# EnricoMiccoli/nodal

Measured on NVIDIA B200. Metric: unknowns_per_second, higher is better.
Workload: dtype f64

## Files before the change

### nodal_b200/csrc/amg.cu

```cuda
#include <algorithm>
#include <cmath>

#include "amg_host.cuh"

void amg_free_csr(nodal_ctx* ctx, AmgCsr& a) {
    if (a.owned) {
        ctx_pool_free(ctx, const_cast<int32_t*>(a.indptr));
        ctx_pool_free(ctx, const_cast<int32_t*>(a.indices));
        ctx_pool_free(ctx, const_cast<double*>(a.data));
    }
    a = AmgCsr();
}

int amg_aggregate(nodal_ctx* ctx, int rounds, const AmgCsr& A, int32_t nown, int32_t base,
                  int32_t** agg_out, int32_t* nc_out, cudaStream_t st) {
    const int32_t n = A.n;
    AmgScratch<int32_t> match(ctx, n), best(ctx, n);
    AmgScratch<u32> leader(ctx, n);
    if (!match.ptr || !best.ptr || !leader.ptr) return NODAL_CUDA_ERROR;
    const int grid = amg_rows_grid(ctx, n);
    CUDA_TRY(cudaMemsetAsync(match, 0xFF, sizeof(int32_t) * (size_t)n, st));
    for (int r = 0; r < rounds; ++r) {
        amg_propose_kernel<<<grid, AT, 0, st>>>(n, A.indptr, A.indices, A.data, match, best, nown, base);
        KERNEL_CHECK();
        amg_accept_kernel<<<grid, AT, 0, st>>>(n, best, match);
        KERNEL_CHECK();
    }
    int32_t* root = best;
    amg_root_kernel<<<grid, AT, 0, st>>>(n, A.indptr, A.indices, A.data, match, root, leader, nown, base);
    KERNEL_CHECK();
    NODAL_TRY(ctx_reserve(ctx, scan_scratch_bytes(n) + 4096));
    u32* total = carve<u32>(ctx, 16);
    if (!total) return NODAL_CUDA_ERROR;
    NODAL_TRY(scan_exclusive_u32(ctx, leader, leader, n, total, st));
    int32_t* agg = match;
    amg_assign_kernel<<<grid, AT, 0, st>>>(n, root, leader, agg);
    KERNEL_CHECK();
    u32* total_h = reinterpret_cast<u32*>(ctx->pinned);
    CUDA_TRY(cudaMemcpyAsync(total_h, total, sizeof(u32), cudaMemcpyDeviceToHost, st));
    CUDA_TRY(cudaStreamSynchronize(st));
    *nc_out = (int32_t)total_h[0];
    *agg_out = match.keep();
    return NODAL_OK;
}

int amg_transpose_pattern(nodal_ctx* ctx, int32_t n, const int32_t* agg, int32_t** pt_ptr_out,
                          int32_t** pt_idx_out, cudaStream_t st) {
    AmgScratch<u64> keys(ctx, n);
    AmgScratch<double> vals(ctx, n), rhs(ctx, (size_t)n + 1), ones(ctx, n);
    if (!keys.ptr || !vals.ptr || !rhs.ptr || !ones.ptr) return NODAL_CUDA_ERROR;
    const int cb = amg_bit_length(n);
    amg_pt_keys_kernel<<<amg_rows_grid(ctx, n), AT, 0, st>>>(n, agg, cb, keys, vals);
    KERNEL_CHECK();
    int64_t cnt = 0;
    NODAL_TRY(nodal_csr_build(ctx, n, n, cb, reinterpret_cast<uint64_t*>(keys.ptr), vals, rhs, &cnt, st));
    if (cnt != n) {
        nodal_set_error("amg: internal error, P^T has %lld entries for %d rows", (long long)cnt, n);
        return NODAL_CUDA_ERROR;
    }
    AmgScratch<int32_t> pp(ctx, (size_t)n + 1), pi(ctx, n);
    if (!pp.ptr || !pi.ptr) return NODAL_CUDA_ERROR;
    NODAL_TRY(nodal_csr_fetch(ctx, n, n, pp, pi, ones, st));
    *pt_ptr_out = pp.keep();
    *pt_idx_out = pi.keep();
    return NODAL_OK;
}

int amg_members(nodal_ctx* ctx, int32_t n, const int32_t* agg, int32_t nc, int32_t** pt_ptr_out,
                int32_t** pt_idx_out, cudaStream_t st) {
    AmgScratch<u32> cnt(ctx, (size_t)nc + 1), cursor(ctx, (size_t)nc + 1);
    AmgScratch<int32_t> pp(ctx, (size_t)nc + 1), pi(ctx, (size_t)std::max(n, 1));
    if (!cnt.ptr || !cursor.ptr || !pp.ptr || !pi.ptr) return NODAL_CUDA_ERROR;
    CUDA_TRY(cudaMemsetAsync(cnt, 0, sizeof(u32) * ((size_t)nc + 1), st));
    CUDA_TRY(cudaMemsetAsync(cursor, 0, sizeof(u32) * ((size_t)nc + 1), st));
    const int grid = amg_rows_grid(ctx, n);
    amg_count_members_kernel<<<grid, AT, 0, st>>>(n, agg, cnt);
    KERNEL_CHECK();
    NODAL_TRY(ctx_reserve(ctx, scan_scratch_bytes((int64_t)nc + 1) + 4096));
    NODAL_TRY(scan_exclusive_u32(ctx, cnt, reinterpret_cast<u32*>(pp.ptr), (int64_t)nc + 1, nullptr, st));
    amg_place_members_kernel<<<grid, AT, 0, st>>>(n, agg, pp, cursor, pi);
    KERNEL_CHECK();
    amg_sort_members_kernel<<<amg_rows_grid(ctx, nc), AT, 0, st>>>(nc, pp, pi);
    KERNEL_CHECK();
    *pt_ptr_out = pp.keep();
    *pt_idx_out = pi.keep();
    return NODAL_OK;
}

int amg_galerkin_merge(nodal_ctx* ctx, const AmgCsr& A, const int32_t* pt_ptr, const int32_t* pt_idx, int32_t nc,
                       const int32_t* label, int32_t ncol_limit, AmgCsr* out, cudaStream_t st) {
    if (A.nnz >= ((int64_t)1 << 32) - 1) return NODAL_BAD_ARG;
    AmgScratch<u32> bound(ctx, (size_t)nc + 1), kept(ctx, (size_t)nc + 1);
    AmgScratch<int32_t> tmp_cols(ctx, (size_t)std::max<int64_t>(A.nnz, 1)), ip(ctx, (size_t)nc + 1);
    AmgScratch<double> tmp_vals(ctx, (size_t)std::max<int64_t>(A.nnz, 1));
    if (!bound.ptr || !kept.ptr || !tmp_cols.ptr || !tmp_vals.ptr || !ip.ptr) return NODAL_CUDA_ERROR;
    const int grid = amg_rows_grid(ctx, nc);
    CUDA_TRY(cudaMemsetAsync(bound.ptr + nc, 0, sizeof(u32), st));
    CUDA_TRY(cudaMemsetAsync(kept.ptr + nc, 0, sizeof(u32), st));
    amg_merge_bound_kernel<<<grid, AT, 0, st>>>(nc, pt_ptr, pt_idx, A.indptr, bound);
    KERNEL_CHECK();
    NODAL_TRY(ctx_reserve(ctx, scan_scratch_bytes((int64_t)nc + 1) + 4096));
    u32* total = carve<u32>(ctx, 16);
    if (!total) return NODAL_CUDA_ERROR;
    const size_t mark = ctx->arena_used;
    NODAL_TRY(scan_exclusive_u32(ctx, bound, bound, (int64_t)nc + 1, nullptr, st));
    ctx->arena_used = mark;
    amg_merge_rows_kernel<<<grid, AT, 0, st>>>(nc, pt_ptr, pt_idx, A.indptr, A.indices, A.data, label, ncol_limit,
                                               bound, tmp_cols, tmp_vals, kept);
    KERNEL_CHECK();
    NODAL_TRY(scan_exclusive_u32(ctx, kept, reinterpret_cast<u32*>(ip.ptr), (int64_t)nc + 1, total, st));
    u32* total_h = reinterpret_cast<u32*>(ctx->pinned);
    CUDA_TRY(cudaMemcpyAsync(total_h, total, sizeof(u32), cudaMemcpyDeviceToHost, st));
    CUDA_TRY(cudaStreamSynchronize(st));
    const int64_t nnzc = total_h[0];
    AmgScratch<int32_t> ix(ctx, (size_t)std::max<int64_t>(nnzc, 1));
    AmgScratch<double> dv(ctx, (size_t)std::max<int64_t>(nnzc, 1));
    if (!ix.ptr || !dv.ptr) return NODAL_CUDA_ERROR;
    amg_merge_compact_kernel<<<grid, AT, 0, st>>>(nc, bound, ip, tmp_cols, tmp_vals, ix, dv);
    KERNEL_CHECK();
    out->n = nc;
    out->nnz = nnzc;
    out->indptr = ip.keep();
    out->indices = ix.keep();
    out->data = dv.keep();
    out->owned = true;
    return NODAL_OK;
}

namespace {

int rows_grid(const nodal_ctx* ctx, int64_t work) { return amg_rows_grid(ctx, work); }
int sell_grid(const nodal_ctx* ctx, int32_t nslices) { return amg_sell_grid(ctx, nslices); }
int bit_length(int64_t v) { return amg_bit_length(v); }
template <typename T>
T* pool(nodal_ctx* ctx, size_t count) { return amg_pool<T>(ctx, count); }
template <typename T>
using Scratch = AmgScratch<T>;
using Csr = AmgCsr;
void free_csr(nodal_ctx* ctx, Csr& a) { amg_free_csr(ctx, a); }
int aggregate(nodal_amg* h, const Csr& A, int32_t** agg_out, int32_t* nc_out, cudaStream_t st) {
    return amg_aggregate(h->ctx, h->rounds, A, 0x7fffffff, 0, agg_out, nc_out, st);
}

bool sorted_galerkin() {
    static const bool on = getenv("NODAL_AMG_SORT_GALERKIN") != nullptr;
    return on;
}

int galerkin(nodal_amg* h, const Csr& A, const int32_t* agg, int32_t nc, Csr* out, cudaStream_t st) {
    nodal_ctx* ctx = h->ctx;
    if (!sorted_galerkin() && amg_merge_pays(A.nnz, nc)) {
        int32_t *pp = nullptr, *pi = nullptr;
        NODAL_TRY(amg_members(ctx, A.n, agg, nc, &pp, &pi, st));
        const int rc = amg_galerkin_merge(ctx, A, pp, pi, nc, agg, 0x7fffffff, out, st);
        ctx_pool_free(ctx, pp);
        ctx_pool_free(ctx, pi);
        return rc;
    }
    Scratch<u64> keys(ctx, A.nnz);
    Scratch<double> vals(ctx, A.nnz), rhs(ctx, (size_t)nc + 1);
    if (!keys.ptr || !vals.ptr || !rhs.ptr) return NODAL_CUDA_ERROR;
    const int cb = bit_length(nc);
    amg_relabel_kernel<<<rows_grid(ctx, A.n), AT, 0, st>>>(A.n, A.indptr, A.indices, A.data, agg, cb,
                                                         keys, vals);
    KERNEL_CHECK();
    int64_t nnzc = 0;
    NODAL_TRY(nodal_csr_build(ctx, nc, A.nnz, cb, reinterpret_cast<uint64_t*>(keys.ptr), vals, rhs,
                              &nnzc, st));
    Scratch<int32_t> ip(ctx, (size_t)nc + 1), ix(ctx, nnzc);
    Scratch<double> dv(ctx, nnzc);
    if (!ip.ptr || !ix.ptr || !dv.ptr) return NODAL_CUDA_ERROR;
    NODAL_TRY(nodal_csr_fetch(ctx, nc, nnzc, ip, ix, dv, st));
    out->n = nc;
    out->nnz = nnzc;
    out->indptr = ip.keep();
    out->indices = ix.keep();
    out->data = dv.keep();
    out->owned = true;
    return NODAL_OK;
}

int transpose_pattern(nodal_amg* h, AmgLevel& L, cudaStream_t st) {
    if (!sorted_galerkin()) return amg_members(h->ctx, L.n, L.agg, L.nc, &L.pt_ptr, &L.pt_idx, st);
    return amg_transpose_pattern(h->ctx, L.n, L.agg, &L.pt_ptr, &L.pt_idx, st);
}

int invert_coarsest(nodal_amg* h, const AmgLevel& L, cudaStream_t st) {
    nodal_ctx* ctx = h->ctx;
    const int32_t n = L.n;
    const size_t elems = (size_t)n * 2 * n;
    Scratch<double> m0(ctx, elems + 32), m1(ctx, elems);
    if (!m0.ptr || !m1.ptr) return NODAL_CUDA_ERROR;
    int* bad = reinterpret_cast<int*>(m0.ptr + elems);
    CUDA_TRY(cudaMemsetAsync(m0, 0, sizeof(double) * (elems + 32), st));
    amg_dense_init_kernel<<<rows_grid(ctx, n), AT, 0, st>>>(n, L.indptr, L.indices, L.data, m0);
    KERNEL_CHECK();
    double *src = m0.ptr, *dst = m1.ptr;
    const int grid = rows_grid(ctx, (int64_t)elems);
    for (int32_t k = 0; k < n; ++k) {
        amg_gj_step_kernel<<<grid, AT, 0, st>>>(n, k, src, dst, bad);
        KERNEL_CHECK();
        std::swap(src, dst);
    }
    h->inv = pool<double>(ctx, (size_t)n * n);
    if (!h->inv) return NODAL_CUDA_ERROR;
    amg_dense_extract_kernel<<<rows_grid(ctx, (int64_t)n * n), AT, 0, st>>>(n, src, h->inv);
    KERNEL_CHECK();
    int* bad_h = reinterpret_cast<int*>(ctx->pinned);
    CUDA_TRY(cudaMemcpyAsync(bad_h, bad, sizeof(int), cudaMemcpyDeviceToHost, st));
    CUDA_TRY(cudaStreamSynchronize(st));
    if (*bad_h != 0) {
        nodal_set_error("amg: the coarsest operator is not positive definite (pivot %d of %d); "
                        "the matrix is not SPD", *bad_h, n);
        return NODAL_BREAKDOWN;
    }
    return NODAL_OK;
}

int build_hierarchy(nodal_amg* h, int32_t n, int64_t nnz, const int32_t* indptr, const int32_t* indices,
                    const double* data, cudaStream_t st) {
    nodal_ctx* ctx = h->ctx;
    Csr cur;
    cur.n = n; cur.nnz = nnz; cur.indptr = indptr; cur.indices = indices; cur.data = data;
    while (cur.n > h->coarse && (int)h->lv.size() < h->maxlevels) {
        Csr A = cur;
        A.owned = false;
        int32_t* comp = nullptr;
        int rc = NODAL_OK;
        for (int pass = 0; pass < h->passes && rc == NODAL_OK; ++pass) {
            int32_t* agg = nullptr;
            int32_t nc = 0;
            Csr Ac;
            rc = aggregate(h, A, &agg, &nc, st);
            if (rc == NODAL_OK) rc = galerkin(h, A, agg, nc, &Ac, st);
            if (rc == NODAL_OK && comp) {
                amg_compose_kernel<<<rows_grid(ctx, cur.n), AT, 0, st>>>(cur.n, comp, agg);
                ++g_nodal_launches;
                if (cudaGetLastError() != cudaSuccess) {
                    nodal_set_error("amg: amg_compose_kernel launch failed");
                    rc = NODAL_CUDA_ERROR;
                }
            }
            if (!comp) comp = agg;
            else ctx_pool_free(ctx, agg);
            free_csr(ctx, A);
            A = Ac;
        }
        double total_nnz = (double)cur.nnz + (double)A.nnz;
        for (const AmgLevel& P : h->lv) total_nnz += (double)P.nnz;
        const bool too_dense = (double)A.nnz > h->max_fill * (double)cur.nnz ||
                               total_nnz > h->max_complexity * (double)(h->lv.empty() ? cur.nnz : h->lv[0].nnz);
        if (rc != NODAL_OK || (double)A.n > 0.9 * (double)cur.n || too_dense) {
            free_csr(ctx, A);
            ctx_pool_free(ctx, comp);
            if (rc != NODAL_OK) {
                free_csr(ctx, cur);
                return rc;
            }
            break;
        }
        AmgLevel L;
        L.n = cur.n; L.nnz = cur.nnz; L.indptr = cur.indptr; L.indices = cur.indices; L.data = cur.data;
        L.owned = cur.owned;
        L.agg = comp;
        L.nc = A.n;
        h->lv.push_back(L);
        cur = A;
        rc = transpose_pattern(h, h->lv.back(), st);
        if (rc != NODAL_OK) {
            free_csr(ctx, cur);
            return rc;
        }
    }
    AmgLevel L;
    L.n = cur.n; L.nnz = cur.nnz; L.indptr = cur.indptr; L.indices = cur.indices; L.data = cur.data;
    L.owned = cur.owned;
    h->lv.push_back(L);
    for (size_t l = 0; l < h->lv.size(); ++l) {
        AmgLevel& V = h->lv[l];
        NODAL_TRY(sell_from_csr(ctx, V.n, V.nnz, V.indptr, V.indices, V.data, &V.sell, st, nullptr));
        V.x = pool<double>(ctx, V.n);
        V.r = pool<double>(ctx, V.n);
        if (l > 0) V.b = pool<double>(ctx, V.n);
        if (!V.x || !V.r || (l > 0 && !V.b)) return NODAL_CUDA_ERROR;
    }
    if (h->lv.back().n <= h->direct_max) NODAL_TRY(invert_coarsest(h, h->lv.back(), st));
    return NODAL_OK;
}

template <int MODE>
int sell_sweep(const nodal_amg* h, const AmgLevel& V, const double* b, const double* x, double* y,
               double* part, cudaStream_t st) {
    const nodal_sell* m = V.sell;
    amg_sell_kernel<MODE><<<sell_grid(h->ctx, m->nslices), AT, 0, st>>>(
        m->n, m->nslices, m->slice_w, m->cols, m->vals, m->dinv, b, x, h->omega, y, part);
    KERNEL_CHECK();
    return NODAL_OK;
}

template <int MODE>
int cycle_sweep(const nodal_amg* h, const AmgLevel& V, const double* b, const double* xc, double* y,
                cudaStream_t st) {
    const nodal_sell* m = V.sell;
    amg_cycle_sweep_kernel<MODE><<<sell_grid(h->ctx, m->nslices), AT, 0, st>>>(
        m->n, m->nslices, m->slice_w, m->cols, m->vals, m->dinv, b, h->omega, V.agg, xc, h->scale, y);
    KERNEL_CHECK();
    return NODAL_OK;
}

int cycle(const nodal_amg* h, const double* b0, double* z0, cudaStream_t st) {
    const nodal_ctx* ctx = h->ctx;
    const int last = (int)h->lv.size() - 1;
    for (int l = 0; l < last; ++l) {
        const AmgLevel& V = h->lv[l];
        const double* b = l == 0 ? b0 : V.b;
        NODAL_TRY(cycle_sweep<1>(h, V, b, nullptr, V.r, st));
        amg_restrict_kernel<<<rows_grid(ctx, V.nc), AT, 0, st>>>(V.nc, V.pt_ptr, V.pt_idx, V.r,
                                                              h->lv[l + 1].b);
        KERNEL_CHECK();
    }
    {
        const AmgLevel& V = h->lv[last];
        const double* b = last == 0 ? b0 : V.b;
        double* x = last == 0 ? z0 : V.x;
        if (h->inv) amg_gemv_kernel<<<rows_grid(ctx, (int64_t)V.n * 32), AT, 0, st>>>(V.n, h->inv, b, x);
        else amg_jacobi0_kernel<<<rows_grid(ctx, V.n), AT, 0, st>>>(V.n, V.sell->dinv, b, h->omega, x);
        KERNEL_CHECK();
    }
    for (int l = last - 1; l >= 0; --l) {
        const AmgLevel& V = h->lv[l];
        const double* b = l == 0 ? b0 : V.b;
        NODAL_TRY(cycle_sweep<2>(h, V, b, h->lv[l + 1].x, l == 0 ? z0 : V.x, st));
    }
    return NODAL_OK;
}

}

extern "C" int nodal_amg_destroy(nodal_amg* h) {
    if (!h) return NODAL_OK;
    cudaSetDevice(h->device);
    nodal_ctx* ctx = h->ctx;
    for (AmgLevel& V : h->lv) {
        sell_free(V.sell);
        if (V.owned) {
            ctx_pool_free(ctx, const_cast<int32_t*>(V.indptr));
            ctx_pool_free(ctx, const_cast<int32_t*>(V.indices));
            ctx_pool_free(ctx, const_cast<double*>(V.data));
        }
        ctx_pool_free(ctx, V.agg);
        ctx_pool_free(ctx, V.pt_ptr);
        ctx_pool_free(ctx, V.pt_idx);
        ctx_pool_free(ctx, V.b);
        ctx_pool_free(ctx, V.x);
        ctx_pool_free(ctx, V.r);
    }
    ctx_pool_free(ctx, h->inv);
    ctx_pool_free(ctx, h->p);
    ctx_pool_free(ctx, h->q);
    ctx_pool_free(ctx, h->r);
    ctx_pool_free(ctx, h->z);
    ctx_pool_free(ctx, h->part);
    delete h;
    return NODAL_OK;
}

extern "C" int nodal_amg_create(nodal_ctx* ctx, int32_t n, int64_t nnz, const int32_t* indptr,
                                const int32_t* indices, const double* data, const double* params,
                                nodal_amg** out, void* stream) {
    NvtxRange nvtx_range("nodal_amg_create");
    if (!ctx || n < 0 || nnz < 0 || !out) return NODAL_BAD_ARG;
    *out = nullptr;
    cudaStream_t st = (cudaStream_t)stream;
    CUDA_TRY(cudaSetDevice(ctx->device));
    nodal_amg* h = new nodal_amg();
    h->ctx = ctx;
    h->device = ctx->device;
    if (params) {
        if (params[0] >= 1.0) h->passes = (int)params[0];
        if (params[1] >= 1.0) h->coarse = (int)params[1];
        if (params[2] > 0.0) h->omega = params[2];
        if (params[3] > 0.0) h->scale = params[3];
        if (params[4] >= 1.0) h->maxlevels = (int)params[4];
        if (params[5] >= 1.0) h->rounds = (int)params[5];
        if (params[6] >= 1.0) h->direct_max = (int)params[6];
        if (params[7] > 0.0) h->max_fill = params[7];
    }
    cudaEvent_t e0, e1;
    CUDA_TRY(cudaEventCreate(&e0));
    CUDA_TRY(cudaEventCreate(&e1));
    cudaEventRecord(e0, st);
    int rc = NODAL_OK;
    if (n > 0) rc = build_hierarchy(h, n, nnz, indptr, indices, data, st);
    if (rc == NODAL_OK && n > 0) {
        h->nparts = std::max(sell_grid(ctx, h->lv[0].sell->nslices), rows_grid(ctx, n));
        h->p = pool<double>(ctx, n);
        h->q = pool<double>(ctx, n);
        h->r = pool<double>(ctx, n);
        h->z = pool<double>(ctx, n);
        h->part = pool<double>(ctx, 3 * (size_t)h->nparts + 16);
        if (!h->p || !h->q || !h->r || !h->z || !h->part) rc = NODAL_CUDA_ERROR;
    }
    cudaEventRecord(e1, st);
    if (cudaEventSynchronize(e1) == cudaSuccess) cudaEventElapsedTime(&h->setup_ms, e0, e1);
    cudaEventDestroy(e0);
    cudaEventDestroy(e1);
    if (rc != NODAL_OK) {
        nodal_amg_destroy(h);
        return rc;
    }
    *out = h;
    return NODAL_OK;
}

extern "C" int nodal_amg_info(const nodal_amg* h, int32_t cap, int32_t* nlevels, int64_t* rows,
                              int64_t* nnz, double* setup_ms, int32_t* direct) {
    if (!h || !nlevels) return NODAL_BAD_ARG;
    *nlevels = (int32_t)h->lv.size();
    for (int32_t l = 0; l < *nlevels && l < cap; ++l) {
        if (rows) rows[l] = h->lv[l].n;
        if (nnz) nnz[l] = h->lv[l].nnz;
    }
    if (setup_ms) *setup_ms = h->setup_ms;
    if (direct) *direct = h->inv ? 1 : 0;
    return NODAL_OK;
}

extern "C" int nodal_amg_fetch_level(nodal_ctx* ctx, const nodal_amg* h, int32_t level, int32_t* agg,
                                     int32_t* indptr, int32_t* indices, double* data, void* stream) {
    if (!ctx || !h || level < 0 || level >= (int32_t)h->lv.size()) return NODAL_BAD_ARG;
    cudaStream_t st = (cudaStream_t)stream;
    CUDA_TRY(cudaSetDevice(ctx->device));
    const AmgLevel& V = h->lv[level];
    if (agg) {
        if (!V.agg) return NODAL_BAD_ARG;
        CUDA_TRY(cudaMemcpyAsync(agg, V.agg, sizeof(int32_t) * (size_t)V.n, cudaMemcpyDeviceToDevice, st));
    }
    if (indptr) CUDA_TRY(cudaMemcpyAsync(indptr, V.indptr, sizeof(int32_t) * ((size_t)V.n + 1), cudaMemcpyDeviceToDevice, st));
    if (indices) CUDA_TRY(cudaMemcpyAsync(indices, V.indices, sizeof(int32_t) * (size_t)V.nnz, cudaMemcpyDeviceToDevice, st));
    if (data) CUDA_TRY(cudaMemcpyAsync(data, V.data, sizeof(double) * (size_t)V.nnz, cudaMemcpyDeviceToDevice, st));
    return NODAL_OK;
}

extern "C" int nodal_amg_apply(nodal_ctx* ctx, const nodal_amg* h, const double* r, double* z,
                               void* stream) {
    if (!ctx || !h || h->ctx != ctx) return NODAL_BAD_ARG;
    if (h->lv.empty()) return NODAL_OK;
    CUDA_TRY(cudaSetDevice(ctx->device));
    return cycle(h, r, z, (cudaStream_t)stream);
}

extern "C" int nodal_amg_pcg(nodal_ctx* ctx, nodal_amg* h, const double* rhs, double* x, double rtol,
                             int32_t maxit, int32_t* iters_h, double* relres_h, double* stats_h,
                             void* stream) {
    NvtxRange nvtx_range("nodal_amg_pcg");
    if (!ctx || !h || h->ctx != ctx || !iters_h || !relres_h) return NODAL_BAD_ARG;
    *iters_h = 0;
    *relres_h = 0.0;
    if (stats_h) memset(stats_h, 0, 16 * sizeof(double));
    if (h->lv.empty()) return NODAL_OK;
    cudaStream_t st = (cudaStream_t)stream;
    CUDA_TRY(cudaSetDevice(ctx->device));
    const AmgLevel& A = h->lv[0];
    const int32_t n = A.n;
    const int gv = rows_grid(ctx, n);
    const int gs = sell_grid(ctx, A.sell->nslices);
    double* part_pq = h->part;
    double* part_rr = h->part + h->nparts;
    double* part_rz = h->part + 2 * (size_t)h->nparts;
    double* scal = h->part + 3 * (size_t)h->nparts;
    double* host = reinterpret_cast<double*>(ctx->pinned);
    cudaEvent_t e0, e1;
    CUDA_TRY(cudaEventCreate(&e0));
    CUDA_TRY(cudaEventCreate(&e1));
    int iters = 0, restarts = 0, rc = NODAL_NOT_CONVERGED;
    double relres = 0.0;
    bool timed = false;

    auto dot_to_host = [&](const double* a, const double* b, double* result) -> int {
        apcg_dot_kernel<<<gv, AT, 0, st>>>(n, a, b, part_rr);
        KERNEL_CHECK();
        apcg_sum_kernel<<<1, AT, 0, st>>>(part_rr, gv, scal + 2);
        KERNEL_CHECK();
        CUDA_TRY(cudaMemcpyAsync(host, scal + 2, sizeof(double), cudaMemcpyDeviceToHost, st));
        CUDA_TRY(cudaStreamSynchronize(st));
        *result = host[0];
        return NODAL_OK;
    };
    auto run = [&]() -> int {
        CUDA_TRY(cudaEventRecord(e0, st));
        double bb = 0.0, rr = 0.0;
        NODAL_TRY(dot_to_host(rhs, rhs, &bb));
        if (!(bb > 0.0)) {
            if (bb == 0.0) {
                CUDA_TRY(cudaMemsetAsync(x, 0, sizeof(double) * (size_t)n, st));
                rc = NODAL_OK;
                return NODAL_OK;
            }
            nodal_set_error("nodal_amg_pcg: the right-hand side is not finite");
            rc = NODAL_BREAKDOWN;
            return NODAL_OK;
        }
        const double bnorm = sqrt(bb);
        NODAL_TRY(sell_sweep<1>(h, A, rhs, x, h->r, nullptr, st));
        NODAL_TRY(dot_to_host(h->r, h->r, &rr));
        relres = sqrt(rr) / bnorm;
        while (true) {
            if (relres <= rtol) { rc = NODAL_OK; break; }
            if (iters >= maxit) { rc = NODAL_NOT_CONVERGED; break; }
            if (restarts > 8) { rc = NODAL_NOT_CONVERGED; break; }
            int par = 0;
            NODAL_TRY(cycle(h, h->r, h->z, st));
            apcg_dot_kernel<<<gv, AT, 0, st>>>(n, h->r, h->z, part_rz);
            KERNEL_CHECK();
            apcg_direction_kernel<<<gv, AT, 0, st>>>(n, part_rz, gv, scal + (par ^ 1), scal + par, h->z, h->p, 1);
            KERNEL_CHECK();
            bool broke = false;
            while (iters < maxit) {
                NODAL_TRY(sell_sweep<0>(h, A, nullptr, h->p, h->q, part_pq, st));
                apcg_update_kernel<<<gv, AT, 0, st>>>(n, part_pq, gs, scal + par, h->p, h->q, x, h->r, part_rr);
                KERNEL_CHECK();
                apcg_sum_kernel<<<1, AT, 0, st>>>(part_rr, gv, scal + 2);
                KERNEL_CHECK();
                CUDA_TRY(cudaMemcpyAsync(host, scal + 2, sizeof(double), cudaMemcpyDeviceToHost, st));
                CUDA_TRY(cudaStreamSynchronize(st));
                ++iters;
                rr = host[0];
                if (!std::isfinite(rr)) { broke = true; break; }
                if (sqrt(rr) <= rtol * bnorm) break;
                NODAL_TRY(cycle(h, h->r, h->z, st));
                apcg_dot_kernel<<<gv, AT, 0, st>>>(n, h->r, h->z, part_rz);
                KERNEL_CHECK();
                apcg_direction_kernel<<<gv, AT, 0, st>>>(n, part_rz, gv, scal + par, scal + (par ^ 1), h->z, h->p, 0);
                KERNEL_CHECK();
                par ^= 1;
            }
            if (broke) {
                nodal_set_error("nodal_amg_pcg: breakdown (non-finite residual) at iteration %d", iters);
                rc = NODAL_BREAKDOWN;
                break;
            }
            NODAL_TRY(sell_sweep<1>(h, A, rhs, x, h->r, nullptr, st));
            NODAL_TRY(dot_to_host(h->r, h->r, &rr));
            relres = sqrt(rr) / bnorm;
            if (!std::isfinite(relres)) { rc = NODAL_BREAKDOWN; break; }
            if (relres > rtol) ++restarts;
        }
        CUDA_TRY(cudaEventRecord(e1, st));
        CUDA_TRY(cudaEventSynchronize(e1));
        timed = true;
        return NODAL_OK;
    };
    const int st_run = run();
    float ms = 0.f;
    if (st_run == NODAL_OK && timed) cudaEventElapsedTime(&ms, e0, e1);
    cudaEventDestroy(e0);
    cudaEventDestroy(e1);
    if (st_run != NODAL_OK) return st_run;
    *iters_h = iters;
    *relres_h = relres;
    if (stats_h) {
        double rows = 0.0, nnz = 0.0;
        for (const AmgLevel& V : h->lv) { rows += V.n; nnz += (double)V.nnz; }
        stats_h[0] = (double)h->lv.size();
        stats_h[1] = A.nnz ? nnz / (double)A.nnz : 0.0;
        stats_h[2] = restarts;
        stats_h[3] = ms;
        stats_h[4] = h->setup_ms;
        stats_h[5] = h->lv.back().n;
        stats_h[6] = n ? rows / n : 0.0;
        stats_h[7] = h->inv ? 1.0 : 0.0;
    }
    return rc;
}

extern "C" int nodal_amg_profile_sweeps(nodal_ctx* ctx, nodal_amg* h, int32_t reps, double* ms_out, void* stream) {
    if (!ctx || !h || h->ctx != ctx || !ms_out || reps < 1 || h->lv.empty()) return NODAL_BAD_ARG;
    cudaStream_t st = (cudaStream_t)stream;
    CUDA_TRY(cudaSetDevice(ctx->device));
    const AmgLevel& A = h->lv[0];
    CUDA_TRY(cudaMemsetAsync(h->p, 0, sizeof(double) * (size_t)A.n, st));
    CUDA_TRY(cudaMemsetAsync(h->r, 0, sizeof(double) * (size_t)A.n, st));
    cudaEvent_t e0, e1;
    CUDA_TRY(cudaEventCreate(&e0));
    CUDA_TRY(cudaEventCreate(&e1));
    int rc = NODAL_OK;
    for (int mode = 0; mode < 3 && rc == NODAL_OK; ++mode) {
        for (int k = -2; k < reps && rc == NODAL_OK; ++k) {
            if (k == 0) cudaEventRecord(e0, st);
            if (mode == 0) rc = sell_sweep<0>(h, A, nullptr, h->p, h->q, h->part, st);
            if (mode == 1) rc = sell_sweep<1>(h, A, h->r, h->p, h->q, nullptr, st);
            if (mode == 2) rc = sell_sweep<2>(h, A, h->r, h->p, h->q, nullptr, st);
        }
        cudaEventRecord(e1, st);
        float ms = 0.f;
        if (cudaEventSynchronize(e1) == cudaSuccess) cudaEventElapsedTime(&ms, e0, e1);
        ms_out[mode] = ms / reps;
    }
    cudaEventDestroy(e0);
    cudaEventDestroy(e1);
    return rc;
}

extern "C" int nodal_amg_profile_cycle(nodal_ctx* ctx, nodal_amg* h, int32_t reps, double* ms_out, void* stream) {
    if (!ctx || !h || h->ctx != ctx || !ms_out || reps < 1 || h->lv.size() < 2) return NODAL_BAD_ARG;
    cudaStream_t st = (cudaStream_t)stream;
    CUDA_TRY(cudaSetDevice(ctx->device));
    const AmgLevel& A = h->lv[0];
    const AmgLevel& C = h->lv[1];
    double* b = h->r;
    CUDA_TRY(cudaMemsetAsync(b, 0, sizeof(double) * (size_t)A.n, st));
    CUDA_TRY(cudaMemsetAsync(A.x, 0, sizeof(double) * (size_t)A.n, st));
    CUDA_TRY(cudaMemsetAsync(C.x, 0, sizeof(double) * (size_t)C.n, st));
    cudaEvent_t e0, e1;
    CUDA_TRY(cudaEventCreate(&e0));
    CUDA_TRY(cudaEventCreate(&e1));
    int rc = NODAL_OK;
    for (int k = 0; k < 6 && rc == NODAL_OK; ++k) {
        for (int i = -2; i < reps && rc == NODAL_OK; ++i) {
            if (i == 0) cudaEventRecord(e0, st);
            switch (k) {
                case 0:
                    amg_jacobi0_kernel<<<rows_grid(ctx, A.n), AT, 0, st>>>(A.n, A.sell->dinv, b, h->omega, A.x);
                    KERNEL_CHECK();
                    break;
                case 1: rc = sell_sweep<1>(h, A, b, A.x, A.r, nullptr, st); break;
                case 2:
                    amg_prolong_kernel<<<rows_grid(ctx, A.n), AT, 0, st>>>(A.n, A.agg, C.x, h->scale, A.x, A.r);
                    KERNEL_CHECK();
                    break;
                case 3: rc = sell_sweep<2>(h, A, b, A.r, h->z, nullptr, st); break;
                case 4: rc = cycle_sweep<1>(h, A, b, nullptr, A.r, st); break;
                default: rc = cycle_sweep<2>(h, A, b, C.x, h->z, st); break;
            }
        }
        cudaEventRecord(e1, st);
        float ms = 0.f;
        if (cudaEventSynchronize(e1) == cudaSuccess) cudaEventElapsedTime(&ms, e0, e1);
        ms_out[k] = ms / reps;
    }
    cudaEventDestroy(e0);
    cudaEventDestroy(e1);
    return rc;
}
```

### nodal_b200/csrc/amg_kernels.cuh

```cuda
#pragma once
#include "amg_core.cuh"
#include "amg_merge_core.cuh"
#include "sparse.cuh"

constexpr int AT = 256;

#define ROW_LOOP(i, n)                                                              \
    for (int64_t i = (int64_t)blockIdx.x * blockDim.x + threadIdx.x; i < (int64_t)(n); \
         i += (int64_t)gridDim.x * blockDim.x)

static __global__ void __launch_bounds__(AT)
amg_propose_kernel(int32_t n, const int32_t* __restrict__ indptr, const int32_t* __restrict__ indices,
                   const double* __restrict__ data, const int32_t* __restrict__ match,
                   int32_t* __restrict__ best, int32_t nown, int32_t base) {
    ROW_LOOP(i, n) best[i] = match[i] >= 0 ? -1 : amg_pick((int32_t)i, indptr, indices, data, match, nown, base);
}

static __global__ void __launch_bounds__(AT)
amg_accept_kernel(int32_t n, const int32_t* __restrict__ best, int32_t* __restrict__ match) {
    ROW_LOOP(i, n) {
        if (match[i] >= 0) continue;
        const int32_t b = best[i];
        if (b >= 0 && best[b] == (int32_t)i) match[i] = b;
    }
}

static __global__ void __launch_bounds__(AT)
amg_root_kernel(int32_t n, const int32_t* __restrict__ indptr, const int32_t* __restrict__ indices,
                const double* __restrict__ data, const int32_t* __restrict__ match,
                int32_t* __restrict__ root, u32* __restrict__ leader, int32_t nown, int32_t base) {
    ROW_LOOP(i, n) {
        const int32_t r = amg_root((int32_t)i, indptr, indices, data, match, nown, base);
        root[i] = r;
        leader[i] = r == (int32_t)i ? 1u : 0u;
    }
}

static __global__ void __launch_bounds__(AT)
amg_assign_kernel(int32_t n, const int32_t* __restrict__ root, const u32* __restrict__ ids,
                  int32_t* __restrict__ agg) {
    ROW_LOOP(i, n) agg[i] = (int32_t)ids[root[i]];
}

static __global__ void __launch_bounds__(AT)
amg_compose_kernel(int32_t n, int32_t* __restrict__ comp, const int32_t* __restrict__ next) {
    ROW_LOOP(i, n) comp[i] = next[comp[i]];
}

static __global__ void __launch_bounds__(AT)
amg_relabel_kernel(int32_t n, const int32_t* __restrict__ indptr, const int32_t* __restrict__ indices,
                   const double* __restrict__ data, const int32_t* __restrict__ agg, int cb,
                   u64* __restrict__ keys, double* __restrict__ vals) {
    ROW_LOOP(i, n) {
        const u64 hi = (u64)agg[i] << cb;
        const int32_t e = indptr[i + 1];
        for (int32_t p = indptr[i]; p < e; ++p) {
            keys[p] = hi | (u64)agg[indices[p]];
            vals[p] = data[p];
        }
    }
}

static __global__ void __launch_bounds__(AT)
amg_pt_keys_kernel(int32_t n, const int32_t* __restrict__ agg, int cb, u64* __restrict__ keys,
                   double* __restrict__ vals) {
    ROW_LOOP(i, n) {
        keys[i] = ((u64)agg[i] << cb) | (u64)i;
        vals[i] = 1.0;
    }
}

static __global__ void __launch_bounds__(AT)
amg_dense_init_kernel(int32_t n, const int32_t* __restrict__ indptr, const int32_t* __restrict__ indices,
                      const double* __restrict__ data, double* __restrict__ M) {
    const int64_t W = 2 * (int64_t)n;
    ROW_LOOP(i, n) {
        M[i * W + n + i] = 1.0;
        const int32_t e = indptr[i + 1];
        for (int32_t p = indptr[i]; p < e; ++p) M[i * W + indices[p]] = data[p];
    }
}

static __global__ void __launch_bounds__(AT)
amg_gj_step_kernel(int32_t n, int32_t k, const double* __restrict__ src, double* __restrict__ dst,
                   int* __restrict__ bad) {
    const int64_t W = 2 * (int64_t)n;
    const double piv = src[k * W + k];
    if (blockIdx.x == 0 && threadIdx.x == 0 && !(piv > 0.0) && *bad == 0) *bad = k + 1;
    ROW_LOOP(idx, (int64_t)n * W) {
        const int64_t i = idx / W, j = idx - i * W;
        const double rkj = src[k * W + j] / piv;
        dst[idx] = i == k ? rkj : src[idx] - src[i * W + k] * rkj;
    }
}

static __global__ void __launch_bounds__(AT)
amg_dense_extract_kernel(int32_t n, const double* __restrict__ M, double* __restrict__ inv) {
    const int64_t W = 2 * (int64_t)n;
    ROW_LOOP(idx, (int64_t)n * n) {
        const int64_t i = idx / n, j = idx - i * n;
        inv[idx] = M[i * W + n + j];
    }
}

static __global__ void __launch_bounds__(AT)
amg_gemv_kernel(int32_t n, const double* __restrict__ inv, const double* __restrict__ b,
                double* __restrict__ x) {
    const int lane = threadIdx.x & 31;
    const int64_t warp = ((int64_t)blockIdx.x * blockDim.x + threadIdx.x) >> 5;
    const int64_t nwarps = ((int64_t)gridDim.x * blockDim.x) >> 5;
    for (int64_t r = warp; r < n; r += nwarps) {
        double acc = 0.0;
        for (int32_t j = lane; j < n; j += 32) acc = fma(inv[r * n + j], b[j], acc);
        acc = warp_sum(acc);
        if (lane == 0) x[r] = acc;
    }
}

static __global__ void __launch_bounds__(AT)
amg_jacobi0_kernel(int32_t n, const double* __restrict__ dinv, const double* __restrict__ b,
                   double omega, double* __restrict__ x) {
    ROW_LOOP(i, n) x[i] = amg_jacobi_start(omega, dinv[i], b[i]);
}

template <int MODE>
static __global__ void __launch_bounds__(AT, 5)
amg_sell_kernel(int32_t n, int32_t nslices, const u32* __restrict__ slice_w,
                const int32_t* __restrict__ cols, const double* __restrict__ vals,
                const double* __restrict__ dinv, const double* __restrict__ b,
                const double* __restrict__ x, double omega, double* __restrict__ y,
                double* __restrict__ part) {
    __shared__ double red[33];
    const int lane = threadIdx.x & 31;
    const int64_t warp = ((int64_t)blockIdx.x * blockDim.x + threadIdx.x) >> 5;
    const int64_t nwarps = ((int64_t)gridDim.x * blockDim.x) >> 5;
    double dot = 0.0;
    for (int64_t s = warp; s < nslices; s += nwarps) {
        const u32 w0 = slice_w[s];
        const int w = (int)(slice_w[s + 1] - w0);
        const double acc = sell_row_dot(cols, vals, (int64_t)w0 * 32 + lane, w, x);
        const int64_t r = s * 32 + lane;
        if (r < n) {
            if (MODE == 0) { y[r] = acc; dot = fma(x[r], acc, dot); }
            if (MODE == 1) y[r] = amg_residual(b[r], acc);
            if (MODE == 2) y[r] = amg_jacobi_update(omega, dinv[r], b[r], acc, x[r]);
        }
    }
    if (MODE == 0) {
        const double t = block_sum(dot, red);
        if (threadIdx.x == 0) part[blockIdx.x] = t;
    }
}

static __global__ void __launch_bounds__(AT)
amg_restrict_kernel(int32_t nc, const int32_t* __restrict__ pt_ptr, const int32_t* __restrict__ pt_idx,
                    const double* __restrict__ r, double* __restrict__ bc) {
    ROW_LOOP(I, nc) {
        double s = 0.0;
        const int32_t e = pt_ptr[I + 1];
        for (int32_t p = pt_ptr[I]; p < e; ++p) s += r[pt_idx[p]];
        bc[I] = s;
    }
}

static __global__ void __launch_bounds__(AT)
amg_prolong_kernel(int32_t n, const int32_t* __restrict__ agg, const double* __restrict__ xc,
                   double scale, const double* __restrict__ x, double* __restrict__ xa) {
    ROW_LOOP(i, n) xa[i] = amg_prolong_add(scale, xc[agg[i]], x[i]);
}

struct JacobiStartAt {
    const double* __restrict__ dinv;
    const double* __restrict__ b;
    double omega;
    __device__ __forceinline__ double operator()(int32_t c) const {
        return amg_jacobi_start(omega, __ldg(&dinv[c]), __ldg(&b[c]));
    }
};

struct ProlongatedAt {
    JacobiStartAt x0;
    const int32_t* __restrict__ agg;
    const double* __restrict__ xc;
    double scale;
    __device__ __forceinline__ double operator()(int32_t c) const {
        return amg_prolong_add(scale, __ldg(&xc[__ldg(&agg[c])]), x0(c));
    }
};

template <int MODE>
static __global__ void __launch_bounds__(AT, 5)
amg_cycle_sweep_kernel(int32_t n, int32_t nslices, const u32* __restrict__ slice_w,
                       const int32_t* __restrict__ cols, const double* __restrict__ vals,
                       const double* __restrict__ dinv, const double* __restrict__ b, double omega,
                       const int32_t* __restrict__ agg, const double* __restrict__ xc, double scale,
                       double* __restrict__ y) {
    const int lane = threadIdx.x & 31;
    const int64_t warp = ((int64_t)blockIdx.x * blockDim.x + threadIdx.x) >> 5;
    const int64_t nwarps = ((int64_t)gridDim.x * blockDim.x) >> 5;
    const JacobiStartAt x0{dinv, b, omega};
    const ProlongatedAt xa{x0, agg, xc, scale};
    for (int64_t s = warp; s < nslices; s += nwarps) {
        const u32 w0 = slice_w[s];
        const int w = (int)(slice_w[s + 1] - w0);
        const int64_t base = (int64_t)w0 * 32 + lane;
        const int64_t r = s * 32 + lane;
        if (MODE == 1) {
            const double acc = sell_row_gather(cols, vals, base, w, x0);
            if (r < n) y[r] = amg_residual(b[r], acc);
        }
        if (MODE == 2) {
            const double acc = sell_row_gather(cols, vals, base, w, xa);
            if (r < n) y[r] = amg_jacobi_update(omega, dinv[r], b[r], acc, xa((int32_t)r));
        }
    }
}

static __global__ void __launch_bounds__(AT)
apcg_dot_kernel(int32_t n, const double* __restrict__ a, const double* __restrict__ b,
                double* __restrict__ part) {
    __shared__ double red[33];
    double t = 0.0;
    ROW_LOOP(i, n) t = fma(a[i], b[i], t);
    t = block_sum(t, red);
    if (threadIdx.x == 0) part[blockIdx.x] = t;
}

static __global__ void __launch_bounds__(AT)
apcg_sum_kernel(const double* __restrict__ part, int count, double* __restrict__ out) {
    __shared__ double red[33];
    const double t = reduce_partials(part, count, red);
    if (threadIdx.x == 0) out[0] = t;
}

static __global__ void __launch_bounds__(AT)
apcg_update_kernel(int32_t n, const double* __restrict__ part_pq, int npq, const double* __restrict__ rz,
                   const double* __restrict__ p, const double* __restrict__ q, double* __restrict__ x,
                   double* __restrict__ r, double* __restrict__ part_rr) {
    __shared__ double red[33];
    const double pq = reduce_partials(part_pq, npq, red);
    const double alpha = rz[0] / pq;
    double t = 0.0;
    ROW_LOOP(i, n) {
        x[i] = fma(alpha, p[i], x[i]);
        const double ri = fma(-alpha, q[i], r[i]);
        r[i] = ri;
        t = fma(ri, ri, t);
    }
    t = block_sum(t, red);
    if (threadIdx.x == 0) part_rr[blockIdx.x] = t;
}

static __global__ void __launch_bounds__(AT)
apcg_direction_kernel(int32_t n, const double* __restrict__ part_rz, int nrz,
                      const double* __restrict__ rz_old, double* __restrict__ rz_new,
                      const double* __restrict__ z, double* __restrict__ p, int first) {
    __shared__ double red[33];
    const double rzn = reduce_partials(part_rz, nrz, red);
    const double beta = first ? 0.0 : rzn / rz_old[0];
    ROW_LOOP(i, n) p[i] = first ? z[i] : fma(beta, p[i], z[i]);
    if (blockIdx.x == 0 && threadIdx.x == 0) rz_new[0] = rzn;
}


static __global__ void __launch_bounds__(AT)
amg_count_members_kernel(int32_t n, const int32_t* __restrict__ agg, u32* __restrict__ cnt) {
    ROW_LOOP(i, n) atomicAdd(&cnt[agg[i]], 1u);
}

static __global__ void __launch_bounds__(AT)
amg_place_members_kernel(int32_t n, const int32_t* __restrict__ agg, const int32_t* __restrict__ pt_ptr,
                         u32* __restrict__ cursor, int32_t* __restrict__ pt_idx) {
    ROW_LOOP(i, n) {
        const int32_t a = agg[i];
        pt_idx[pt_ptr[a] + (int32_t)atomicAdd(&cursor[a], 1u)] = (int32_t)i;
    }
}

static __global__ void __launch_bounds__(AT)
amg_sort_members_kernel(int32_t nc, const int32_t* __restrict__ pt_ptr, int32_t* __restrict__ pt_idx) {
    ROW_LOOP(I, nc) {
        const int32_t b = pt_ptr[I], e = pt_ptr[I + 1];
        for (int32_t p = b + 1; p < e; ++p) {
            const int32_t v = pt_idx[p];
            int32_t q = p;
            while (q > b && pt_idx[q - 1] > v) { pt_idx[q] = pt_idx[q - 1]; --q; }
            pt_idx[q] = v;
        }
    }
}

static __global__ void __launch_bounds__(AT)
amg_merge_bound_kernel(int32_t nc, const int32_t* __restrict__ pt_ptr, const int32_t* __restrict__ pt_idx,
                       const int32_t* __restrict__ indptr, u32* __restrict__ bound) {
    ROW_LOOP(I, nc) bound[I] = (u32)amg_merge_bound((int32_t)I, pt_ptr, pt_idx, indptr);
}

static __global__ void __launch_bounds__(AT)
amg_merge_rows_kernel(int32_t nc, const int32_t* __restrict__ pt_ptr, const int32_t* __restrict__ pt_idx,
                      const int32_t* __restrict__ indptr, const int32_t* __restrict__ indices,
                      const double* __restrict__ data, const int32_t* __restrict__ label, int32_t ncol_limit,
                      const u32* __restrict__ off, int32_t* tmp_cols, double* tmp_vals, u32* __restrict__ kept) {
    constexpr int LOCAL = 32;
    ROW_LOOP(I, nc) {
        const u32 o = off[I];
        if (off[I + 1] - o <= (u32)LOCAL) {
            int32_t lc[LOCAL];
            double lv[LOCAL];
            const int32_t k = amg_merge_row((int32_t)I, pt_ptr, pt_idx, indptr, indices, data, label, lc, lv, ncol_limit);
            for (int32_t e = 0; e < k; ++e) { tmp_cols[o + e] = lc[e]; tmp_vals[o + e] = lv[e]; }
            kept[I] = (u32)k;
        } else {
            kept[I] = (u32)amg_merge_row((int32_t)I, pt_ptr, pt_idx, indptr, indices, data, label, tmp_cols + o,
                                         tmp_vals + o, ncol_limit);
        }
    }
}

static __global__ void __launch_bounds__(AT)
amg_merge_compact_kernel(int32_t nc, const u32* __restrict__ off, const int32_t* __restrict__ out_ptr,
                         const int32_t* __restrict__ tmp_cols, const double* __restrict__ tmp_vals,
                         int32_t* __restrict__ out_cols, double* __restrict__ out_vals) {
    ROW_LOOP(I, nc) {
        const int32_t b = out_ptr[I], cnt = out_ptr[I + 1] - b;
        const u32 src = off[I];
        for (int32_t k = 0; k < cnt; ++k) {
            out_cols[b + k] = tmp_cols[src + k];
            out_vals[b + k] = tmp_vals[src + k];
        }
    }
}
```

Before: 145.3 million.

## Fuse Gauss-Jordan steps into one cooperative kernel and early-exit matching rounds

The coarsest-level dense inversion used to launch one kernel per pivot column. It now runs as a single cooperative kernel that loops over pivots with grid-wide syncs, which removes the per-step launch overhead. Aggregation matching rounds now record whether any pair was accepted, and later rounds return immediately once nothing changed. Rows with no candidate partner are marked so later rounds skip them. The cooperative launch limits the grid to resident blocks, and each grid sync adds its own cost.

```diff
diff --git a/nodal_b200/csrc/amg.cu b/nodal_b200/csrc/amg.cu
--- a/nodal_b200/csrc/amg.cu
+++ b/nodal_b200/csrc/amg.cu
@@ -16,14 +16,16 @@
                   int32_t** agg_out, int32_t* nc_out, cudaStream_t st) {
     const int32_t n = A.n;
     AmgScratch<int32_t> match(ctx, n), best(ctx, n);
-    AmgScratch<u32> leader(ctx, n);
-    if (!match.ptr || !best.ptr || !leader.ptr) return NODAL_CUDA_ERROR;
+    AmgScratch<u32> leader(ctx, n), accepted(ctx, (size_t)std::max(rounds, 1));
+    if (!match.ptr || !best.ptr || !leader.ptr || !accepted.ptr) return NODAL_CUDA_ERROR;
     const int grid = amg_rows_grid(ctx, n);
     CUDA_TRY(cudaMemsetAsync(match, 0xFF, sizeof(int32_t) * (size_t)n, st));
+    CUDA_TRY(cudaMemsetAsync(accepted, 0, sizeof(u32) * (size_t)std::max(rounds, 1), st));
     for (int r = 0; r < rounds; ++r) {
-        amg_propose_kernel<<<grid, AT, 0, st>>>(n, A.indptr, A.indices, A.data, match, best, nown, base);
+        const u32* prev = r > 0 ? accepted.ptr + r - 1 : nullptr;
+        amg_propose_kernel<<<grid, AT, 0, st>>>(n, A.indptr, A.indices, A.data, match, best, nown, base, prev);
         KERNEL_CHECK();
-        amg_accept_kernel<<<grid, AT, 0, st>>>(n, best, match);
+        amg_accept_kernel<<<grid, AT, 0, st>>>(n, best, match, prev, accepted.ptr + r);
         KERNEL_CHECK();
     }
     int32_t* root = best;
@@ -195,13 +197,15 @@
     CUDA_TRY(cudaMemsetAsync(m0, 0, sizeof(double) * (elems + 32), st));
     amg_dense_init_kernel<<<rows_grid(ctx, n), AT, 0, st>>>(n, L.indptr, L.indices, L.data, m0);
     KERNEL_CHECK();
-    double *src = m0.ptr, *dst = m1.ptr;
-    const int grid = rows_grid(ctx, (int64_t)elems);
-    for (int32_t k = 0; k < n; ++k) {
-        amg_gj_step_kernel<<<grid, AT, 0, st>>>(n, k, src, dst, bad);
-        KERNEL_CHECK();
-        std::swap(src, dst);
-    }
+    int per_sm = 0;
+    CUDA_TRY(cudaOccupancyMaxActiveBlocksPerMultiprocessor(&per_sm, amg_gauss_jordan_kernel, AT, 0));
+    const int grid = (int)std::min<int64_t>((int64_t)std::max(per_sm, 1) * ctx->num_sms, rows_grid(ctx, (int64_t)elems));
+    int32_t n_ = n;
+    double *a0 = m0.ptr, *a1 = m1.ptr;
+    void* args[] = {&n_, &a0, &a1, &bad};
+    CUDA_TRY(cudaLaunchCooperativeKernel((void*)amg_gauss_jordan_kernel, dim3(grid), dim3(AT), args, 0, st));
+    ++g_nodal_launches;
+    const double* src = n % 2 == 0 ? m0.ptr : m1.ptr;
     h->inv = pool<double>(ctx, (size_t)n * n);
     if (!h->inv) return NODAL_CUDA_ERROR;
     amg_dense_extract_kernel<<<rows_grid(ctx, (int64_t)n * n), AT, 0, st>>>(n, src, h->inv);
diff --git a/nodal_b200/csrc/amg_kernels.cuh b/nodal_b200/csrc/amg_kernels.cuh
--- a/nodal_b200/csrc/amg_kernels.cuh
+++ b/nodal_b200/csrc/amg_kernels.cuh
@@ -3,26 +3,47 @@
 #include "amg_merge_core.cuh"
 #include "sparse.cuh"
 
+#include <cooperative_groups.h>
+namespace cg = cooperative_groups;
+
 constexpr int AT = 256;
 
 #define ROW_LOOP(i, n)                                                              \
     for (int64_t i = (int64_t)blockIdx.x * blockDim.x + threadIdx.x; i < (int64_t)(n); \
          i += (int64_t)gridDim.x * blockDim.x)
 
+constexpr int32_t AMG_NO_PARTNER = -2;
+
 static __global__ void __launch_bounds__(AT)
 amg_propose_kernel(int32_t n, const int32_t* __restrict__ indptr, const int32_t* __restrict__ indices,
-                   const double* __restrict__ data, const int32_t* __restrict__ match,
-                   int32_t* __restrict__ best, int32_t nown, int32_t base) {
-    ROW_LOOP(i, n) best[i] = match[i] >= 0 ? -1 : amg_pick((int32_t)i, indptr, indices, data, match, nown, base);
-}
-
-static __global__ void __launch_bounds__(AT)
-amg_accept_kernel(int32_t n, const int32_t* __restrict__ best, int32_t* __restrict__ match) {
+                   const double* __restrict__ data, int32_t* __restrict__ match, int32_t* __restrict__ best,
+                   int32_t nown, int32_t base, const u32* __restrict__ prev_accepted) {
+    if (prev_accepted && *prev_accepted == 0u) return;
+    ROW_LOOP(i, n) {
+        const int32_t m = match[i];
+        int32_t b = -1;
+        if (m == -1) {
+            b = amg_pick((int32_t)i, indptr, indices, data, match, nown, base);
+            if (b < 0) match[i] = AMG_NO_PARTNER;
+        }
+        best[i] = b;
+    }
+}
+
+static __global__ void __launch_bounds__(AT)
+amg_accept_kernel(int32_t n, const int32_t* __restrict__ best, int32_t* __restrict__ match,
+                  const u32* __restrict__ prev_accepted, u32* accepted) {
+    if (prev_accepted && *prev_accepted == 0u) return;
+    bool any = false;
     ROW_LOOP(i, n) {
         if (match[i] >= 0) continue;
         const int32_t b = best[i];
-        if (b >= 0 && best[b] == (int32_t)i) match[i] = b;
-    }
+        if (b >= 0 && best[b] == (int32_t)i) {
+            match[i] = b;
+            any = true;
+        }
+    }
+    if (__any_sync(0xffffffffu, any) && (threadIdx.x & 31) == 0 && *accepted == 0u) *accepted = 1u;
 }
 
 static __global__ void __launch_bounds__(AT)
@@ -82,15 +103,23 @@
 }
 
 static __global__ void __launch_bounds__(AT)
-amg_gj_step_kernel(int32_t n, int32_t k, const double* __restrict__ src, double* __restrict__ dst,
-                   int* __restrict__ bad) {
+amg_gauss_jordan_kernel(int32_t n, double* m0, double* m1, int* bad) {
+    cg::grid_group grid = cg::this_grid();
     const int64_t W = 2 * (int64_t)n;
-    const double piv = src[k * W + k];
-    if (blockIdx.x == 0 && threadIdx.x == 0 && !(piv > 0.0) && *bad == 0) *bad = k + 1;
-    ROW_LOOP(idx, (int64_t)n * W) {
-        const int64_t i = idx / W, j = idx - i * W;
-        const double rkj = src[k * W + j] / piv;
-        dst[idx] = i == k ? rkj : src[idx] - src[i * W + k] * rkj;
+    const double* src = m0;
+    double* dst = m1;
+    for (int32_t k = 0; k < n; ++k) {
+        const double piv = src[k * W + k];
+        if (blockIdx.x == 0 && threadIdx.x == 0 && !(piv > 0.0) && *bad == 0) *bad = k + 1;
+        ROW_LOOP(idx, (int64_t)n * W) {
+            const int64_t i = idx / W, j = idx - i * W;
+            const double rkj = src[k * W + j] / piv;
+            dst[idx] = i == k ? rkj : src[idx] - src[i * W + k] * rkj;
+        }
+        grid.sync();
+        double* t = const_cast<double*>(src);
+        src = dst;
+        dst = t;
     }
 }
 
```

After: 147.0 million, median of 6. +1.2%, better.

## Fuse Gauss-Jordan steps into one cooperative kernel with grid sync

Applied to the files above, without the earlier changes.

The coarsest-level dense inversion used to launch one kernel per pivot column, n launches in total. It now runs as a single cooperative kernel that loops over pivots and calls grid.sync() between steps, with the grid capped at the number of co-resident blocks. The elimination update also moves to an explicit FMA. This removes per-step launch overhead, at the cost of grid-wide barrier latency and a smaller grid, and the FMA changes rounding slightly. The code only runs during hierarchy setup, so its effect on the solve metric depends on whether setup is timed.

```diff
diff --git a/nodal_b200/csrc/amg.cu b/nodal_b200/csrc/amg.cu
--- a/nodal_b200/csrc/amg.cu
+++ b/nodal_b200/csrc/amg.cu
@@ -195,16 +195,27 @@
     CUDA_TRY(cudaMemsetAsync(m0, 0, sizeof(double) * (elems + 32), st));
     amg_dense_init_kernel<<<rows_grid(ctx, n), AT, 0, st>>>(n, L.indptr, L.indices, L.data, m0);
     KERNEL_CHECK();
-    double *src = m0.ptr, *dst = m1.ptr;
-    const int grid = rows_grid(ctx, (int64_t)elems);
-    for (int32_t k = 0; k < n; ++k) {
-        amg_gj_step_kernel<<<grid, AT, 0, st>>>(n, k, src, dst, bad);
-        KERNEL_CHECK();
-        std::swap(src, dst);
-    }
+    int per_sm = 0;
+    CUDA_TRY(cudaOccupancyMaxActiveBlocksPerMultiprocessor(&per_sm, amg_gauss_jordan_kernel, AT, 0));
+    if (per_sm < 1) {
+        nodal_set_error("amg: the Gauss-Jordan kernel does not fit on the device");
+        return NODAL_CUDA_ERROR;
+    }
+    cudaLaunchConfig_t cfg = {};
+    cudaLaunchAttribute coop[1];
+    coop[0].id = cudaLaunchAttributeCooperative;
+    coop[0].val.cooperative = 1;
+    cfg.gridDim = dim3((unsigned)std::min<int64_t>(rows_grid(ctx, (int64_t)elems), (int64_t)per_sm * ctx->num_sms));
+    cfg.blockDim = dim3(AT);
+    cfg.stream = st;
+    cfg.attrs = coop;
+    cfg.numAttrs = 1;
+    CUDA_TRY(cudaLaunchKernelEx(&cfg, amg_gauss_jordan_kernel, n, m0.ptr, m1.ptr, bad));
+    ++g_nodal_launches;
+    const double* result = (n & 1) ? m1.ptr : m0.ptr;
     h->inv = pool<double>(ctx, (size_t)n * n);
     if (!h->inv) return NODAL_CUDA_ERROR;
-    amg_dense_extract_kernel<<<rows_grid(ctx, (int64_t)n * n), AT, 0, st>>>(n, src, h->inv);
+    amg_dense_extract_kernel<<<rows_grid(ctx, (int64_t)n * n), AT, 0, st>>>(n, result, h->inv);
     KERNEL_CHECK();
     int* bad_h = reinterpret_cast<int*>(ctx->pinned);
     CUDA_TRY(cudaMemcpyAsync(bad_h, bad, sizeof(int), cudaMemcpyDeviceToHost, st));
diff --git a/nodal_b200/csrc/amg_kernels.cuh b/nodal_b200/csrc/amg_kernels.cuh
--- a/nodal_b200/csrc/amg_kernels.cuh
+++ b/nodal_b200/csrc/amg_kernels.cuh
@@ -1,4 +1,6 @@
 #pragma once
+#include <cooperative_groups.h>
+
 #include "amg_core.cuh"
 #include "amg_merge_core.cuh"
 #include "sparse.cuh"
@@ -81,16 +83,25 @@
     }
 }
 
-static __global__ void __launch_bounds__(AT)
-amg_gj_step_kernel(int32_t n, int32_t k, const double* __restrict__ src, double* __restrict__ dst,
-                   int* __restrict__ bad) {
+__device__ __forceinline__ double amg_gj_element(double src_ij, double a_ik, double rkj, bool pivot_row) {
+    return pivot_row ? rkj : __fma_rn(-a_ik, rkj, src_ij);
+}
+
+static __global__ void __launch_bounds__(AT)
+amg_gauss_jordan_kernel(int32_t n, double* m0, double* m1, int* bad) {
+    cooperative_groups::grid_group grid = cooperative_groups::this_grid();
     const int64_t W = 2 * (int64_t)n;
-    const double piv = src[k * W + k];
-    if (blockIdx.x == 0 && threadIdx.x == 0 && !(piv > 0.0) && *bad == 0) *bad = k + 1;
-    ROW_LOOP(idx, (int64_t)n * W) {
-        const int64_t i = idx / W, j = idx - i * W;
-        const double rkj = src[k * W + j] / piv;
-        dst[idx] = i == k ? rkj : src[idx] - src[i * W + k] * rkj;
+    for (int32_t k = 0; k < n; ++k) {
+        const double* src = (k & 1) ? m1 : m0;
+        double* dst = (k & 1) ? m0 : m1;
+        const double piv = src[k * W + k];
+        if (blockIdx.x == 0 && threadIdx.x == 0 && !(piv > 0.0) && *bad == 0) *bad = k + 1;
+        ROW_LOOP(idx, (int64_t)n * W) {
+            const int64_t i = idx / W, j = idx - i * W;
+            const double rkj = src[k * W + j] / piv;
+            dst[idx] = amg_gj_element(src[idx], src[i * W + k], rkj, i == k);
+        }
+        grid.sync();
     }
 }
 
```

After: 145.1 million before, 145.7 million after (median of 6 runs). No clear change (+0.4%).
